# apple/ml-cvnets

Measured on NVIDIA H100. Metric: images/sec training step, MobileViTv2-1.0 bf16 256x256, higher is better.
Workload: dtype bf16

## Files before the change

### ml-cvnets_b200/csrc/gemm_tc.cu

```cuda
#include "common.cuh"
#include <cstdlib>

namespace {

constexpr int TC_BM = 128;
constexpr int TC_BN = 128;
constexpr int TC_BK = 32;
constexpr int TC_STAGE = TC_BM * TC_BK * 2;
constexpr int TC_WBLK = TC_BN * TC_BK * 2;
constexpr int TC_LDO = TC_BN + 8;
constexpr int TC_EPI_THREADS = 256;
constexpr int TC_PRODUCER_WARP = TC_EPI_THREADS / 32;
constexpr int TC_THREADS = TC_EPI_THREADS + 32;
constexpr int TC_XF_THREADS_MAX = 256;
template <int AMODE>
struct XfCfg {
  static constexpr int THREADS = (AMODE == CVB_A_RAW) ? 0 : (AMODE == CVB_A_BNB ? 128 : TC_XF_THREADS_MAX);
  static constexpr int IT = THREADS ? (TC_BM * 4) / THREADS : 1;
};
constexpr int TC_MAX_STAGES = 12;

enum { TEPI_STORE = 0, TEPI_STORE_R = 1, TEPI_SILU_BWD = 2, TEPI_GN_BWD = 3 };

__device__ __forceinline__ uint64_t desc_sw64(uint32_t saddr) { return wgmma_desc(saddr, 16, 512, WG_SW64); }
__device__ __forceinline__ void epi_bar_sync() { asm volatile("bar.sync 1, %0;" ::"n"(TC_EPI_THREADS) : "memory"); }

template <int AMODE, int EPI, bool WRES>
__global__ void __launch_bounds__(TC_THREADS + XfCfg<AMODE>::THREADS, 1)
    pw_gemm_tc_kernel(const __grid_constant__ CUtensorMap tmA, const __grid_constant__ CUtensorMap tmA2, const __grid_constant__ CUtensorMap tmW,
                      const cvb_gemm_args p, int NST) {
  constexpr bool XF = (AMODE != CVB_A_RAW);
  constexpr bool TWO_A = (AMODE == CVB_A_BNB);
  constexpr bool HAS_P = (AMODE == CVB_A_AFF || AMODE == CVB_A_AFF_SILU || AMODE == CVB_A_GN || AMODE == CVB_A_BNB);
  const int tid = threadIdx.x, lane = tid & 31, warp = tid >> 5;
  const int n0 = blockIdx.x * TC_BN;
  const int KT = (p.K + TC_BK - 1) / TC_BK;
  const int m_tiles = (p.M + TC_BM - 1) / TC_BM;
  const int my_tiles = (m_tiles - (int)blockIdx.y + (int)gridDim.y - 1) / (int)gridDim.y;
  const int total = my_tiles * KT;

  extern __shared__ __align__(1024) uint8_t smem_raw[];
  uint8_t* smem = smem_raw + ((1024u - (smem_u32(smem_raw) & 1023u)) & 1023u);
  constexpr int A_BYTES = (TWO_A ? 2 : 1) * TC_STAGE;
  constexpr int RING_STAGE = A_BYTES + (WRES ? 0 : TC_WBLK);
  uint8_t* sW = smem;
  uint8_t* sA = sW + (WRES ? KT * TC_WBLK : 0);
  uint8_t* sO = sA + NST * RING_STAGE;
  float* sP = reinterpret_cast<float*>(sO + TC_BM * TC_LDO * 2);
  __shared__ __align__(8) uint64_t full[TC_MAX_STAGES], empty[TC_MAX_STAGES], ready[TC_MAX_STAGES];
  __shared__ __align__(8) uint64_t wbar;
  __shared__ double s_samp[2][128];

  if (tid == 0) {
    for (int i = 0; i < NST; ++i) { mbar_init(&full[i], 1); mbar_init(&empty[i], 2); mbar_init(&ready[i], XfCfg<AMODE>::THREADS ? XfCfg<AMODE>::THREADS / 32 : 1); }
    mbar_init(&wbar, 1);
    fence_mbar_init();
  }
  if (tid < 128) { s_samp[0][tid] = 0.0; s_samp[1][tid] = 0.0; }
  __syncthreads();
  pdl_wait();
  pdl_trigger();

  if (warp == TC_PRODUCER_WARP) {
    if (lane == 0) {
      if (WRES) {
        mbar_expect_tx(&wbar, (uint32_t)KT * TC_WBLK);
        for (int kt = 0; kt < KT; ++kt) tma_load_2d(sW + kt * TC_WBLK, &tmW, &wbar, kt * TC_BK, n0);
      }
      for (int it = 0; it < total; ++it) {
        const int stage = it % NST;
        if (it >= NST) mbar_wait(&empty[stage], ((it / NST) - 1) & 1);
        const int j = it / KT, kt = it - j * KT;
        const int m0 = ((int)blockIdx.y + j * (int)gridDim.y) * TC_BM;
        mbar_expect_tx(&full[stage], RING_STAGE);
        tma_load_2d(sA + stage * RING_STAGE, &tmA, &full[stage], kt * TC_BK, m0);
        if (TWO_A) tma_load_2d(sA + stage * RING_STAGE + TC_STAGE, &tmA2, &full[stage], kt * TC_BK, m0);
        if (!WRES) tma_load_2d(sA + stage * RING_STAGE + A_BYTES, &tmW, &full[stage], kt * TC_BK, n0);
      }
    }
  } else if (warp > TC_PRODUCER_WARP) {
    if (XF) {
      constexpr int TC_XF_THREADS = XfCfg<AMODE>::THREADS > 0 ? XfCfg<AMODE>::THREADS : 128;
      constexpr int TC_XF_IT = XfCfg<AMODE>::IT;
      const int tt = tid - TC_THREADS;
      const int Kpad = KT * TC_BK;
      if (HAS_P) {
        for (int k = tt; k < Kpad; k += TC_XF_THREADS) {
          const bool ok = k < p.K;
          sP[k] = ok ? p.a_p0[k] : 0.f;
          sP[Kpad + k] = ok ? p.a_p1[k] : 0.f;
          if (AMODE == CVB_A_BNB) sP[2 * Kpad + k] = ok ? p.a_p2[k] : 0.f;
        }
        asm volatile("bar.sync 2, %0;" ::"n"(TC_XF_THREADS) : "memory");
      }
      float tmu[TC_XF_IT], trs[TC_XF_IT];
#pragma unroll
      for (int i = 0; i < TC_XF_IT; ++i) { tmu[i] = 0.f; trs[i] = 1.f; }
      for (int it = 0; it < total; ++it) {
        const int stage = it % NST;
        const int j = it / KT, kt = it - j * KT;
        const int m0 = ((int)blockIdx.y + j * (int)gridDim.y) * TC_BM;
        const int k0 = kt * TC_BK;
        if (AMODE == CVB_A_GN && kt == 0) {
#pragma unroll
          for (int i = 0; i < TC_XF_IT; ++i) {
            const int m = m0 + (tt >> 2) + i * (TC_XF_THREADS / 4);
            const int b = (m < p.M ? m : p.M - 1) / p.rows_per_sample;
            tmu[i] = __ldg(p.row_mean + b);
            trs[i] = __ldg(p.row_rstd + b);
          }
        }
        mbar_wait(&full[stage], (it / NST) & 1);
        uint8_t* st = sA + stage * RING_STAGE;
#pragma unroll
        for (int i = 0; i < TC_XF_IT; ++i) {
          const int c = tt + i * TC_XF_THREADS;
          const int row = c >> 2, ch = c & 3;
          const int k = k0 + ch * 8;
          const uint32_t off = (uint32_t)(row * 64 + ((ch ^ ((row >> 1) & 3)) << 4));
          uint4* pa = reinterpret_cast<uint4*>(st + off);
          float f[8], q0[8], q1[8];
          unpack8(*pa, f);
          if (HAS_P) {
            *reinterpret_cast<float4*>(q0) = *reinterpret_cast<const float4*>(sP + k);
            *reinterpret_cast<float4*>(q0 + 4) = *reinterpret_cast<const float4*>(sP + k + 4);
            *reinterpret_cast<float4*>(q1) = *reinterpret_cast<const float4*>(sP + Kpad + k);
            *reinterpret_cast<float4*>(q1 + 4) = *reinterpret_cast<const float4*>(sP + Kpad + k + 4);
          }
          if (AMODE == CVB_A_AFF) {
#pragma unroll
            for (int e = 0; e < 8; ++e) f[e] = fmaf(q0[e], f[e], q1[e]);
          } else if (AMODE == CVB_A_AFF_SILU) {
#pragma unroll
            for (int e = 0; e < 8; ++e) f[e] = silu_f(fmaf(q0[e], f[e], q1[e]));
          } else if (AMODE == CVB_A_SILU) {
#pragma unroll
            for (int e = 0; e < 8; ++e) f[e] = silu_f(f[e]);
          } else if (AMODE == CVB_A_GN) {
#pragma unroll
            for (int e = 0; e < 8; ++e) f[e] = fmaf((f[e] - tmu[i]) * trs[i], q0[e], q1[e]);
          } else if (AMODE == CVB_A_BNB) {
            float y[8], q2[8];
            unpack8(*reinterpret_cast<const uint4*>(st + TC_STAGE + off), y);
            *reinterpret_cast<float4*>(q2) = *reinterpret_cast<const float4*>(sP + 2 * Kpad + k);
            *reinterpret_cast<float4*>(q2 + 4) = *reinterpret_cast<const float4*>(sP + 2 * Kpad + k + 4);
#pragma unroll
            for (int e = 0; e < 8; ++e) f[e] = fmaf(q0[e], f[e], fmaf(q1[e], y[e], q2[e]));
          }
          *pa = (m0 + row < p.M) ? pack8(f) : make_uint4(0u, 0u, 0u, 0u);
        }
        fence_proxy_async();
        __syncwarp();
        if (lane == 0) mbar_arrive(&ready[stage]);
      }
    }
  } else {
    const int et = tid;
    const int wg = tid >> 7;
    const int r0 = wg * 64 + ((tid & 127) >> 5) * 16 + (lane >> 2);
    const int pc = 2 * (lane & 3);
    int chn[2];
    bool ch_ok[2];
    float bias[2], ep0[2], ep1[2];
#pragma unroll
    for (int h = 0; h < 2; ++h) {
      chn[h] = n0 + r0 + 8 * h;
      ch_ok[h] = chn[h] < p.N;
      bias[h] = (ch_ok[h] && p.bias) ? __ldg(p.bias + chn[h]) : 0.f;
      ep0[h] = ((EPI == TEPI_SILU_BWD || EPI == TEPI_GN_BWD) && ch_ok[h] && p.e_p0) ? __ldg(p.e_p0 + chn[h]) : 1.f;
      ep1[h] = (EPI == TEPI_SILU_BWD && ch_ok[h] && p.e_p1) ? __ldg(p.e_p1 + chn[h]) : 0.f;
    }
    constexpr bool has_aux = (EPI != TEPI_STORE);
    const bf16* __restrict__ AUX = static_cast<const bf16*>(EPI == TEPI_STORE_R ? p.R : p.Y);
    const int ldaux = EPI == TEPI_STORE_R ? p.ldr : p.ldy;
    const bool want_samp = (p.samp_sum != nullptr) && (EPI != TEPI_GN_BWD);
    const bool lin_bwd = (p.e_mode == CVB_E_LIN_BWD);
    const int rps = p.rows_per_sample > 0 ? p.rows_per_sample : 1;
    float cs[2] = {0.f, 0.f}, cq[2] = {0.f, 0.f};
    bf16* __restrict__ Cg = static_cast<bf16*>(p.C);
    constexpr int CGS = TC_BN / 8;
    const uint32_t w_off = (uint32_t)wg * 64 * 64;

    auto issue_aux = [&](int j) {
      const int m0 = ((int)blockIdx.y + j * (int)gridDim.y) * TC_BM;
      for (int c = et; c < TC_BM * CGS; c += TC_EPI_THREADS) {
        const int row = c / CGS, cgc = c % CGS;
        const int m = m0 + row, n = n0 + cgc * 8;
        const bool ok = (m < p.M) && (n < p.N);
        cp_async16(smem_u32(sO + row * (TC_LDO * 2) + cgc * 16), AUX + (ok ? (size_t)m * ldaux + n : 0), ok);
      }
      cp_async_commit();
    };
    if (has_aux && my_tiles > 0) issue_aux(0);
    if (WRES) mbar_wait(&wbar, 0);

    float acc[64];
    int it = 0;
    for (int j = 0; j < my_tiles; ++j) {
      const int m0 = ((int)blockIdx.y + j * (int)gridDim.y) * TC_BM;
      for (int kt = 0; kt < KT; ++kt, ++it) {
        const int stage = it % NST;
        mbar_wait(XF ? &ready[stage] : &full[stage], (it / NST) & 1);
        const uint32_t aa = smem_u32(sA + stage * RING_STAGE);
        const uint32_t wa = (WRES ? smem_u32(sW + kt * TC_WBLK) : aa + A_BYTES) + w_off;
        wgmma_fence();
#pragma unroll
        for (int k = 0; k < TC_BK / 16; ++k) wgmma_m64n128<0, 0>(acc, desc_sw64(wa + k * 32), desc_sw64(aa + k * 32), (kt | k) ? 1u : 0u);
        wgmma_commit();
        wgmma_wait<1>();
        if (kt > 0 && (tid & 127) == 0) mbar_arrive(&empty[(it - 1) % NST]);
      }
      wgmma_wait<0>();
      wgmma_reg_fence<64>(acc);
      if ((tid & 127) == 0) mbar_arrive(&empty[(it - 1) % NST]);

      if (has_aux) {
        cp_async_wait<0>();
        epi_bar_sync();
      }
      const bool full_tile = (m0 + TC_BM <= p.M);
      float gs[2][2] = {{0.f, 0.f}, {0.f, 0.f}}, gq[2][2] = {{0.f, 0.f}, {0.f, 0.f}};
#pragma unroll
      for (int h = 0; h < 2; ++h) {
        bf16* so = reinterpret_cast<bf16*>(sO) + r0 + 8 * h;
        if (full_tile && !has_aux) {
#pragma unroll
          for (int jb = 0; jb < 16; ++jb) {
#pragma unroll
            for (int e = 0; e < 2; ++e) {
              const float v = acc[4 * jb + 2 * h + e] + bias[h];
              so[(8 * jb + pc + e) * TC_LDO] = __float2bfloat16_rn(v);
              cs[h] += v;
              cq[h] = fmaf(v, v, cq[h]);
            }
          }
        } else {
#pragma unroll
          for (int jb = 0; jb < 16; ++jb) {
#pragma unroll
            for (int e = 0; e < 2; ++e) {
              const int i = 8 * jb + pc + e;
              float v = acc[4 * jb + 2 * h + e] + ((full_tile || m0 + i < p.M) ? bias[h] : 0.f);
              float y = 0.f;
              if (has_aux) y = __bfloat162float(so[i * TC_LDO]);
              if (EPI == TEPI_STORE_R) v += y;
              if (EPI == TEPI_SILU_BWD && !lin_bwd) v *= silu_grad_f(fmaf(ep0[h], y, ep1[h]));
              if (EPI == TEPI_GN_BWD) {
                gs[h][jb >> 3] += v;
                gq[h][jb >> 3] = fmaf(v, y, gq[h][jb >> 3]);
                so[i * TC_LDO] = __float2bfloat16_rn(v * ep0[h]);
              } else {
                const bf16 vb = __float2bfloat16_rn(v);
                so[i * TC_LDO] = vb;
                const float vr = __bfloat162float(vb);
                cs[h] += vr;
                cq[h] = fmaf(vr, EPI == TEPI_SILU_BWD ? y : vr, cq[h]);
              }
            }
          }
        }
      }
      if (EPI == TEPI_GN_BWD) {
        const int nsamples = (p.M + rps - 1) / rps;
#pragma unroll
        for (int h = 0; h < 2; ++h) {
#pragma unroll
          for (int hf = 0; hf < 2; ++hf) {
            float a = gs[h][hf], bx = gq[h][hf];
            a += __shfl_xor_sync(0xffffffffu, a, 1);
            a += __shfl_xor_sync(0xffffffffu, a, 2);
            bx += __shfl_xor_sync(0xffffffffu, bx, 1);
            bx += __shfl_xor_sync(0xffffffffu, bx, 2);
            const int mh = m0 + hf * 64;
            if ((lane & 3) == 0 && ch_ok[h] && mh < p.M) {
              double* wsA = p.gn_ws + (size_t)(mh / rps) * p.N + chn[h];
              atomicAdd(wsA, (double)a);
              atomicAdd(wsA + (size_t)nsamples * p.N, (double)bx);
            }
          }
        }
      }
      epi_bar_sync();
      const int first_sample = m0 / rps;
      for (int c = et; c < TC_BM * CGS; c += TC_EPI_THREADS) {
        const int row = c / CGS, cgc = c % CGS;
        const int m = m0 + row, n = n0 + cgc * 8;
        const uint4 u = *reinterpret_cast<const uint4*>(sO + row * (TC_LDO * 2) + cgc * 16);
        if (m < p.M && n < p.N) stg16(Cg + (size_t)m * p.ldc + n, u);
        if (want_samp) {
          float f[8];
          unpack8(u, f);
          float sv = 0.f, sq = 0.f;
#pragma unroll
          for (int e = 0; e < 8; ++e) { sv += f[e]; sq = fmaf(f[e], f[e], sq); }
#pragma unroll
          for (int o = CGS / 2; o > 0; o >>= 1) {
            sv += __shfl_xor_sync(0xffffffffu, sv, o);
            sq += __shfl_xor_sync(0xffffffffu, sq, o);
          }
          if (cgc == 0 && m < p.M) {
            atomicAdd(&s_samp[0][m / rps - first_sample], (double)sv);
            atomicAdd(&s_samp[1][m / rps - first_sample], (double)sq);
          }
        }
      }
      epi_bar_sync();
      if (want_samp) {
        const int mlast = min(m0 + TC_BM, p.M) - 1;
        const int nsamp = mlast / rps - first_sample + 1;
        if (et < nsamp) {
          atomicAdd(p.samp_sum + first_sample + et, s_samp[0][et]);
          atomicAdd(p.samp_sq + first_sample + et, s_samp[1][et]);
          s_samp[0][et] = 0.0;
          s_samp[1][et] = 0.0;
        }
      }
      if (has_aux && j + 1 < my_tiles) issue_aux(j + 1);
    }
    if (EPI != TEPI_GN_BWD) {
#pragma unroll
      for (int h = 0; h < 2; ++h) {
        float s = cs[h], q = cq[h];
        s += __shfl_xor_sync(0xffffffffu, s, 1);
        s += __shfl_xor_sync(0xffffffffu, s, 2);
        q += __shfl_xor_sync(0xffffffffu, q, 1);
        q += __shfl_xor_sync(0xffffffffu, q, 2);
        if (p.col_sum && ch_ok[h] && (lane & 3) == 0) {
          atomicAdd(p.col_sum + chn[h], (double)s);
          atomicAdd(p.col_sq + chn[h], (double)q);
        }
      }
    }
  }
}

template <int AMODE, int EPI, bool WRES>
int launch_tc_impl(const cvb_gemm_args& a, cudaStream_t st, size_t fixed, int stage_bytes) {
  const size_t budget = (size_t)216 * 1024;
  int nst = (int)((budget - fixed) / stage_bytes);
  if (nst > TC_MAX_STAGES) nst = TC_MAX_STAGES;
  const size_t smem = fixed + (size_t)nst * stage_bytes;
  static bool attr = false;
  if (!attr) {
    CVB_CUDA(cudaFuncSetAttribute(pw_gemm_tc_kernel<AMODE, EPI, WRES>, cudaFuncAttributeMaxDynamicSharedMemorySize, 216 * 1024));
    attr = true;
  }
  const int n_tiles = (a.N + TC_BN - 1) / TC_BN, m_tiles = (a.M + TC_BM - 1) / TC_BM;
  int gy = cvb_num_sms() / n_tiles;
  if (gy > m_tiles) gy = m_tiles;
  if (gy < 1) gy = 1;
  CUtensorMap tmA, tmA2, tmW;
  if (cvb_make_tmap_2d_k32(&tmA, a.A, a.M, a.K, a.lda, TC_BM)) return 1;
  if (cvb_make_tmap_2d_k32(&tmA2, AMODE == CVB_A_BNB ? a.A2 : a.A, a.M, a.K, AMODE == CVB_A_BNB ? a.lda2 : a.lda, TC_BM)) return 1;
  if (cvb_make_tmap_2d_k32(&tmW, a.W, a.N, a.K, a.ldw, TC_BN)) return 1;
  dim3 grid(n_tiles, gy);
  const int threads = TC_THREADS + XfCfg<AMODE>::THREADS;
  CVB_CUDA(cvb_launch(pw_gemm_tc_kernel<AMODE, EPI, WRES>, grid, threads, smem, st, tmA, tmA2, tmW, a, nst));
  CVB_LAUNCH_CHECK();
  return 0;
}

template <int AMODE, int EPI>
int launch_tc(const cvb_gemm_args& a, cudaStream_t st) {
  const int KT = (a.K + TC_BK - 1) / TC_BK;
  const int nvec = (AMODE == CVB_A_AFF || AMODE == CVB_A_AFF_SILU || AMODE == CVB_A_GN) ? 2 : (AMODE == CVB_A_BNB ? 3 : 0);
  const int a_bytes = (AMODE == CVB_A_BNB ? 2 : 1) * TC_STAGE;
  const size_t stagebuf = (size_t)TC_BM * TC_LDO * 2 + (size_t)nvec * KT * TC_BK * 4 + 1024;
  const size_t panel = (size_t)KT * TC_WBLK;
  if (panel + stagebuf + 6 * (size_t)a_bytes <= (size_t)216 * 1024) return launch_tc_impl<AMODE, EPI, true>(a, st, panel + stagebuf, a_bytes);
  return launch_tc_impl<AMODE, EPI, false>(a, st, stagebuf, a_bytes + TC_WBLK);
}

__global__ void __launch_bounds__(128) gn_bwd_ws_finalize_kernel(const double* __restrict__ ws, const float* __restrict__ mean,
                                                                  const float* __restrict__ rstd, const float* __restrict__ gamma, int B, int N,
                                                                  double* col_sum, double* col_sq, double* samp_sum, double* samp_sq) {
  pdl_wait();
  pdl_trigger();
  __shared__ double s_red[2][4];
  const int b = blockIdx.x, tid = threadIdx.x;
  if (b >= B) {
    __shared__ double s_col[2][8][16];
    const int cl = tid & 15, sg = tid >> 4, c = (b - B) * 16 + cl;
    double sa = 0.0, st = 0.0;
    if (c < N) {
#pragma unroll 4
      for (int s = sg; s < B; s += 8) {
        const double A = ws[(size_t)s * N + c], Bx = ws[((size_t)B + s) * N + c];
        sa += A;
        st += (double)rstd[s] * (Bx - (double)mean[s] * A);
      }
    }
    s_col[0][sg][cl] = sa;
    s_col[1][sg][cl] = st;
    __syncthreads();
    if (sg == 0 && c < N) {
      for (int g = 1; g < 8; ++g) { sa += s_col[0][g][cl]; st += s_col[1][g][cl]; }
      col_sum[c] += sa;
      col_sq[c] += st;
    }
    return;
  }
  const double mu = (double)mean[b], rs = (double)rstd[b];
  double sg = 0.0, sgx = 0.0;
  for (int c = tid; c < N; c += 128) {
    const double A = ws[(size_t)b * N + c], Bx = ws[((size_t)B + b) * N + c];
    const double t = rs * (Bx - mu * A);
    const double gm = gamma ? (double)gamma[c] : 1.0;
    sg += gm * A;
    sgx += gm * t;
  }
#pragma unroll
  for (int o = 16; o > 0; o >>= 1) {
    sg += __shfl_xor_sync(0xffffffffu, sg, o);
    sgx += __shfl_xor_sync(0xffffffffu, sgx, o);
  }
  if ((tid & 31) == 0) { s_red[0][tid >> 5] = sg; s_red[1][tid >> 5] = sgx; }
  __syncthreads();
  if (tid == 0 && samp_sum) {
    atomicAdd(samp_sum + b, s_red[0][0] + s_red[0][1] + s_red[0][2] + s_red[0][3]);
    atomicAdd(samp_sq + b, s_red[1][0] + s_red[1][1] + s_red[1][2] + s_red[1][3]);
  }
}

template <int AMODE>
int launch_tc_gn_bwd(const cvb_gemm_args& a, cudaStream_t st) {
  int rc = launch_tc<AMODE, TEPI_GN_BWD>(a, st);
  if (rc != 0) return rc;
  const int B = (a.M + a.rows_per_sample - 1) / a.rows_per_sample;
  const int col_blocks = a.col_sum ? (a.N + 15) / 16 : 0;
  CVB_CUDA(cvb_launch(gn_bwd_ws_finalize_kernel, B + col_blocks, 128, 0, st, static_cast<const double*>(a.gn_ws), a.row_mean, a.row_rstd, a.e_p0, B, a.N, a.col_sum,
                      a.col_sq, a.samp_sum, a.samp_sq));
  CVB_LAUNCH_CHECK();
  return 0;
}

template <int AMODE>
int dispatch_tc_epi(const cvb_gemm_args& a, cudaStream_t st) {
  if (a.e_mode == CVB_E_GN_BWD && a.gn_ws && a.rows_per_sample % (TC_BM / 2) == 0 && !a.bias && (AMODE == CVB_A_RAW || AMODE == CVB_A_BNB))
    return launch_tc_gn_bwd<AMODE == CVB_A_BNB ? CVB_A_BNB : CVB_A_RAW>(a, st);
  if (a.e_mode == CVB_E_STORE) return a.R ? launch_tc<AMODE, TEPI_STORE_R>(a, st) : launch_tc<AMODE, TEPI_STORE>(a, st);
  if ((a.e_mode == CVB_E_SILU_BWD || a.e_mode == CVB_E_LIN_BWD) && (AMODE == CVB_A_RAW || AMODE == CVB_A_BNB)) return launch_tc<AMODE == CVB_A_BNB ? CVB_A_BNB : CVB_A_RAW, TEPI_SILU_BWD>(a, st);
  return -1;
}

}

int cvb_pw_gemm_tc(const cvb_gemm_args& a, cudaStream_t st) {
  static const int min_n = [] { const char* e = getenv("CVB_TC_MIN_N"); return e ? atoi(e) : 96; }();
  if (a.N < min_n || (a.N >= 96 && a.N % 128 != 0 && a.N % 128 < 64 && a.N < 256)) return -1;
  switch (a.a_mode) {
    case CVB_A_RAW: return dispatch_tc_epi<CVB_A_RAW>(a, st);
    case CVB_A_AFF: return dispatch_tc_epi<CVB_A_AFF>(a, st);
    case CVB_A_AFF_SILU: return dispatch_tc_epi<CVB_A_AFF_SILU>(a, st);
    case CVB_A_SILU: return dispatch_tc_epi<CVB_A_SILU>(a, st);
    case CVB_A_GN: return dispatch_tc_epi<CVB_A_GN>(a, st);
    case CVB_A_BNB: return dispatch_tc_epi<CVB_A_BNB>(a, st);
    default: return -1;
  }
}
```

### ml-cvnets_b200/csrc/norm.cu

```cuda
#include <stdarg.h>

#include "common.cuh"

static thread_local char g_err[512] = "";
void cvb_set_error(const char* fmt, ...) {
  va_list ap;
  va_start(ap, fmt);
  vsnprintf(g_err, sizeof(g_err), fmt, ap);
  va_end(ap);
}
extern "C" const char* cvb_last_error(void) { return g_err; }
extern "C" int cvb_abi_version(void) { return CVB_ABI_VERSION; }
static int g_pdl_enabled = 1;
int cvb_pdl_enabled() { return g_pdl_enabled; }
extern "C" int cvb_set_pdl_enabled(int on) {
  int old = g_pdl_enabled;
  g_pdl_enabled = on ? 1 : 0;
  return old;
}

int cvb_num_sms() {
  static int sms = 0;
  if (sms == 0) {
    int dev = 0;
// ... 435 lines not shown
    const float mu = mean[row], rs = rstd[row];
    float v[LNB_MAXCH][8], xh[LNB_MAXCH][8];
    uint4 dres[LNB_MAXCH];
    float s1 = 0.f, s2 = 0.f;
#pragma unroll
    for (int q = 0; q < LNB_MAXCH; ++q) {
      const int ch = lane + 32 * q;
      if (ch < nch) {
        unpack8(ldg16_stream(V + row * C + ch * 8), v[q]);
        unpack8(ldg16_stream(X + row * C + ch * 8), xh[q]);
        if (DRES) dres[q] = ldg16_stream(DRES + row * C + ch * 8);
      }
    }
#pragma unroll
    for (int q = 0; q < LNB_MAXCH; ++q) {
      const int ch = lane + 32 * q;
      if (ch < nch) {
        float gq[8];
        *reinterpret_cast<float4*>(gq) = *reinterpret_cast<const float4*>(sgam + ch * 8);
        *reinterpret_cast<float4*>(gq + 4) = *reinterpret_cast<const float4*>(sgam + ch * 8 + 4);
#pragma unroll
        for (int e = 0; e < 8; ++e) {
          xh[q][e] = (xh[q][e] - mu) * rs;
          atomicAdd(&sred[e * nch + ch], v[q][e]);
          atomicAdd(&sred[C + e * nch + ch], v[q][e] * xh[q][e]);
          v[q][e] *= gq[e];
          s1 += v[q][e];
          s2 = fmaf(v[q][e], xh[q][e], s2);
        }
      }
    }
    s1 = warp_sum(s1) * invC;
    s2 = warp_sum(s2) * invC;
#pragma unroll
    for (int q = 0; q < LNB_MAXCH; ++q) {
      const int ch = lane + 32 * q;
      if (ch < nch) {
        float d[8];
        if (DRES) unpack8(dres[q], d);
#pragma unroll
        for (int e = 0; e < 8; ++e) {
          float o = rs * (v[q][e] - s1 - xh[q][e] * s2);
          if (DRES) o += d[e];
          d[e] = o;
          if (col_sum) atomicAdd(&sred[2 * C + e * nch + ch], o);
        }
        stg16(DX + row * C + ch * 8, pack8(d));
      }
    }
  }
  __syncthreads();
  for (int i = tid; i < C; i += NT) {
    const int t = (i & 7) * (C / 8) + (i >> 3);
    atomicAdd(dbeta + i, (double)sred[t]);
    atomicAdd(dgamma + i, (double)sred[C + t]);
    if (col_sum) atomicAdd(col_sum + i, (double)sred[2 * C + t]);
  }
}

__device__ __forceinline__ float act_fwd_f(float x, int kind) {
  switch (kind) {
    case 0: return silu_f(x);
    case 1: return 0.5f * x * (1.0f + erff(x * 0.70710678118654752f));
    case 2: return fmaxf(x, 0.f);
    case 3: return x * fminf(fmaxf(x + 3.0f, 0.f), 6.0f) * (1.0f / 6.0f);
    case 4: return fminf(fmaxf(x + 3.0f, 0.f), 6.0f) * (1.0f / 6.0f);
    default: return 1.0f / (1.0f + __expf(-x));
  }
}
__device__ __forceinline__ float act_grad_f(float x, int kind) {
  switch (kind) {
    case 0: return silu_grad_f(x);
    case 1: {
      const float cdf = 0.5f * (1.0f + erff(x * 0.70710678118654752f));
      return cdf + x * 0.3989422804014327f * __expf(-0.5f * x * x);
    }
    case 2: return x > 0.f ? 1.f : 0.f;
    case 3: return x <= -3.0f ? 0.f : (x < 3.0f ? fmaf(x, 1.0f / 3.0f, 0.5f) : 1.0f);
    case 4: return (x > -3.0f && x < 3.0f) ? (1.0f / 6.0f) : 0.f;
    default: {
      const float s = 1.0f / (1.0f + __expf(-x));
      return s * (1.0f - s);
    }
  }
}
__global__ void __launch_bounds__(NT) act_fwd_kernel(const bf16* __restrict__ X, bf16* __restrict__ Y, int64_t nvec, int kind) {
  pdl_wait();
  pdl_trigger();
  for (int64_t v = (int64_t)blockIdx.x * NT + threadIdx.x; v < nvec; v += (int64_t)gridDim.x * NT) {
    float f[8];
    unpack8(ldg16_stream(X + v * 8), f);
#pragma unroll
    for (int j = 0; j < 8; ++j) f[j] = act_fwd_f(f[j], kind);
    stg16(Y + v * 8, pack8(f));
  }
}
__global__ void __launch_bounds__(NT) act_bwd_kernel(const bf16* __restrict__ DY, const bf16* __restrict__ X, bf16* __restrict__ DX, int64_t nvec,
                                                     int kind) {
  pdl_wait();
  pdl_trigger();
  for (int64_t v = (int64_t)blockIdx.x * NT + threadIdx.x; v < nvec; v += (int64_t)gridDim.x * NT) {
    float g[8], x[8];
    unpack8(ldg16_stream(DY + v * 8), g);
    unpack8(ldg16_stream(X + v * 8), x);
#pragma unroll
    for (int j = 0; j < 8; ++j) g[j] *= act_grad_f(x[j], kind);
    stg16(DX + v * 8, pack8(g));
  }
}

__global__ void __launch_bounds__(NT) ln_stats_kernel(const bf16* __restrict__ X, int ldx, int64_t M, int C, float eps, float* __restrict__ mean,
                                                      float* __restrict__ rstd) {
  pdl_wait();
  pdl_trigger();
  const int lane = threadIdx.x & 31;
  const int64_t row = (int64_t)blockIdx.x * (NT / 32) + (threadIdx.x >> 5);
  if (row >= M) return;
  const bf16* x = X + row * ldx;
  float s = 0.f, q = 0.f;
  for (int c = lane * 8; c < C; c += 256) {
    float f[8];
    unpack8(ldg16(x + c), f);
#pragma unroll
    for (int e = 0; e < 8; ++e) { s += f[e]; q = fmaf(f[e], f[e], q); }
  }
  s = warp_sum(s);
  q = warp_sum(q);
  if (lane == 0) {
    const float mu = s / (float)C;
    float var = q / (float)C - mu * mu;
    if (var < 0.f) var = 0.f;
    mean[row] = mu;
    rstd[row] = rsqrtf(var + eps);
  }
}

__global__ void __launch_bounds__(NT) gn_bwd_apply_kernel(const bf16* __restrict__ G, const bf16* __restrict__ X, const float* __restrict__ mean,
                                                          const float* __restrict__ rstd, const double* __restrict__ sg, const double* __restrict__ sgx,
                                                          double count, const bf16* __restrict__ DRES, bf16* __restrict__ DX, int64_t M,
                                                          int rows_per_sample, int C, double* col_sum, int cgs, int rpp, int rows_per_cta,
                                                          const float* __restrict__ gamma) {
  pdl_wait();
  pdl_trigger();
  extern __shared__ double sdred[];
  const int tid = threadIdx.x;
  if (col_sum) { for (int i = tid; i < C; i += blockDim.x) sdred[i] = 0.0; __syncthreads(); }
  const int cg = tid % cgs, rr = tid / cgs;
  const int c = cg * 8;
  float a0[8], gm[8];
#pragma unroll
  for (int j = 0; j < 8; ++j) { a0[j] = 0.f; gm[j] = gamma ? gamma[c + j] : 1.0f; }
  int64_t r_begin = (int64_t)blockIdx.x * rows_per_cta, r_end = r_begin + rows_per_cta;
  if (r_end > M) r_end = M;
  for (int64_t r = r_begin + rr; r < r_end; r += rpp) {
    const int b = (int)(r / rows_per_sample);
    const float mu = mean[b], rs = rstd[b];
    const float m1 = (float)(sg[b] / count), m2 = (float)(sgx[b] / count);
    float g[8], x[8];
    unpack8(ldg16_stream(G + r * C + c), g);
    unpack8(ldg16_stream(X + r * C + c), x);
#pragma unroll
    for (int j = 0; j < 8; ++j) {
      float xh = (x[j] - mu) * rs;
      g[j] = rs * (g[j] * gm[j] - m1 - xh * m2);
    }
    if (DRES) {
      float d[8];
      unpack8(ldg16_stream(DRES + r * C + c), d);
#pragma unroll
      for (int j = 0; j < 8; ++j) g[j] += d[j];
    }
#pragma unroll
    for (int j = 0; j < 8; ++j) a0[j] += g[j];
    stg16(DX + r * C + c, pack8(g));
  }
  if (col_sum) {
#pragma unroll
    for (int j = 0; j < 8; ++j) atomicAdd(&sdred[c + j], (double)a0[j]);
    __syncthreads();
    for (int i = tid; i < C; i += blockDim.x) atomicAdd(col_sum + i, sdred[i]);
  }
}

__global__ void __launch_bounds__(NT) pool_fwd_kernel(const bf16* __restrict__ X, int HW, int C, bf16* __restrict__ OUT) {
  pdl_wait();
  pdl_trigger();
  extern __shared__ double sdred[];
  const int b = blockIdx.x;
  const int cgs = C / 8;
  const int tid = threadIdx.x;
  for (int i = tid; i < C; i += blockDim.x) sdred[i] = 0.0;
  __syncthreads();
  const int cg = tid % cgs, rr = tid / cgs, rpp = blockDim.x / cgs;
  float a[8];
#pragma unroll
  for (int j = 0; j < 8; ++j) a[j] = 0.f;
  for (int r = rr; r < HW; r += rpp) {
    float f[8];
    unpack8(ldg16(X + ((int64_t)b * HW + r) * C + cg * 8), f);
#pragma unroll
    for (int j = 0; j < 8; ++j) a[j] += f[j];
  }
#pragma unroll
  for (int j = 0; j < 8; ++j) atomicAdd(&sdred[cg * 8 + j], (double)a[j]);
  __syncthreads();
  for (int i = tid; i < C; i += blockDim.x) OUT[(int64_t)b * C + i] = __float2bfloat16_rn((float)sdred[i] / (float)HW);
}

__global__ void __launch_bounds__(NT) pool_bwd_kernel(const bf16* __restrict__ DOUT, int HW, int C, bf16* __restrict__ DX, int64_t nvec) {
  pdl_wait();
  pdl_trigger();
  const int cgs = C / 8;
  const float inv = 1.f / (float)HW;
  for (int64_t v = (int64_t)blockIdx.x * NT + threadIdx.x; v < nvec; v += (int64_t)gridDim.x * NT) {
    int64_t row = v / cgs;
    int c = (int)(v % cgs) * 8;
    int64_t b = row / HW;
    float f[8];
    unpack8(ldg16(DOUT + b * C + c), f);
#pragma unroll
    for (int j = 0; j < 8; ++j) f[j] *= inv;
    stg16(DX + v * 8, pack8(f));
  }
}

__global__ void __launch_bounds__(NT) stem_im2col_kernel(const float* __restrict__ X, int64_t sxn, int64_t sxc, int64_t sxh, int64_t sxw, int B, int H,
                                                         int W, bf16* __restrict__ A, const float* __restrict__ mix) {
  pdl_wait();
  pdl_trigger();
  const int Ho = H / 2, Wo = W / 2;
  const int mode = mix ? (int)mix[0] : 0;
  const float lam = mix ? mix[1] : 1.f;
  const int bx1 = mix ? (int)mix[2] : 0, by1 = mix ? (int)mix[3] : 0, bx2 = mix ? (int)mix[4] : 0, by2 = mix ? (int)mix[5] : 0;
  const int64_t total = (int64_t)B * Ho * Wo * 4;
  for (int64_t i = (int64_t)blockIdx.x * NT + threadIdx.x; i < total; i += (int64_t)gridDim.x * NT) {
    const int ch = (int)(i & 3);
    const int64_t pix = i >> 2;
    const int ow = (int)(pix % Wo);
    const int oh = (int)((pix / Wo) % Ho);
    const int b = (int)(pix / ((int64_t)Wo * Ho));
    float f[8];
#pragma unroll
    for (int j = 0; j < 8; ++j) {
      const int col = ch * 8 + j;
      float v = 0.f;
      if (col < 27) {
        const int ci = col / 9, u = (col % 9) / 3, vv = col % 3;
        const int h = 2 * oh + u - 1, w = 2 * ow + vv - 1;
        if (h >= 0 && h < H && w >= 0 && w < W) {
          const int64_t off = ci * sxc + h * sxh + w * sxw;
          v = __ldg(X + b * sxn + off);
          if (mode != 0) {
            const int bp = b == 0 ? B - 1 : b - 1;
            if (mode == 1) v = fmaf(lam, v, (1.0f - lam) * __ldg(X + bp * sxn + off));
            else if (h >= by1 && h < by2 && w >= bx1 && w < bx2) v = __ldg(X + bp * sxn + off);
          }
        }
      }
      f[j] = v;
    }
    stg16(A + i * 8, pack8(f));
  }
}

__device__ __forceinline__ int perm_row(int r, int rows, int rot) { return rot ? (r + rot) % rows : r; }

__global__ void __launch_bounds__(NT) prep_weights_kernel(const cvb_prep_desc* __restrict__ descs) {
  pdl_wait();
  pdl_trigger();
  const cvb_prep_desc d = descs[blockIdx.y];
  const int64_t total = (d.kind == 2) ? (int64_t)d.rows * d.cols : (d.kind == 3 ? (int64_t)d.dst_rows : (int64_t)d.dst_rows * d.ldd);
  for (int64_t i = (int64_t)blockIdx.x * NT + threadIdx.x; i < total; i += (int64_t)gridDim.x * NT) {
    if (d.kind == 0) {
      int r = (int)(i / d.ldd), c = (int)(i % d.ldd);
      float v = (r < d.rows && c < d.cols) ? d.src[(int64_t)perm_row(r, d.rows, d.rot) * d.cols + c] : 0.f;
      static_cast<bf16*>(d.dst)[i] = __float2bfloat16_rn(v);
    } else if (d.kind == 1) {
      int c = (int)(i / d.ldd), r = (int)(i % d.ldd);
      float v = (r < d.rows && c < d.cols) ? d.src[(int64_t)perm_row(r, d.rows, d.rot) * d.cols + c] : 0.f;
      static_cast<bf16*>(d.dst)[i] = __float2bfloat16_rn(v);
    } else if (d.kind == 2) {
      int tap = (int)(i / d.rows), ch = (int)(i % d.rows);
      static_cast<float*>(d.dst)[i] = bf16_round(d.src[(int64_t)ch * d.cols + tap]);
    } else if (d.kind == 4 || d.kind == 5) {
      const int r = (d.kind == 4) ? (int)(i / d.ldd) : (int)(i % d.ldd), c = (d.kind == 4) ? (int)(i % d.ldd) : (int)(i / d.ldd);
      const int cin = d.cols / d.rot;
      float v = 0.f;
      if (r < d.rows && c < d.cols) v = d.src[(int64_t)r * d.cols + (c % cin) * d.rot + c / cin];
      static_cast<bf16*>(d.dst)[i] = __float2bfloat16_rn(v);
    } else {
      int r = (int)i;
      static_cast<float*>(d.dst)[i] = (r < d.rows) ? d.src[perm_row(r, d.rows, d.rot)] : 0.f;
    }
  }
}

__global__ void __launch_bounds__(NT) unprep_grad_kernel(const float* __restrict__ src, float* __restrict__ dst, int rows, int cols, int lds, int kind,
                                                         int rot) {
  pdl_wait();
  pdl_trigger();
  const int64_t total = (int64_t)rows * cols;
  for (int64_t i = (int64_t)blockIdx.x * NT + threadIdx.x; i < total; i += (int64_t)gridDim.x * NT) {
    if (kind == 0) {
      int r = (int)(i / cols), c = (int)(i % cols);
      dst[(int64_t)perm_row(r, rows, rot) * cols + c] = src[(int64_t)r * lds + c];
    } else if (kind == 2) {
      int ch = (int)(i / cols), tap = (int)(i % cols);
      dst[i] = src[(int64_t)tap * rows + ch];
    } else if (kind == 4) {
      int r = (int)(i / cols), c = (int)(i % cols);
      const int cin = cols / rot;
      dst[(int64_t)r * cols + (c % cin) * rot + c / cin] = src[(int64_t)r * lds + c];
    } else {
      dst[perm_row((int)i, rows, rot)] = src[i];
    }
  }
}

int grid_for(int64_t n_items) {
  int64_t g = (n_items + NT - 1) / NT;
  int64_t cap = 16 * (int64_t)cvb_num_sms();
  if (g > cap) g = cap;
  if (g < 1) g = 1;
  return (int)g;
}

}

// ... 226 lines not shown
```

Measured before the change: 6882.

## Add 64-row tile variant of pointwise GEMM with two CTAs per SM

Templates the tensor-core pointwise GEMM on the pixel tile height, adding a 64-row variant that uses m64n64 wgmma, half the accumulators, a halved shared-memory budget and two CTAs per SM. Light epilogue GEMMs whose weight panel fits resident now take this path, aiming to improve SM fill and latency hiding on small or skinny problems. Separately, the GroupNorm backward apply kernel is unrolled four rows deep so loads are batched ahead of the math, increasing memory-level parallelism. The smaller tile gives each CTA fewer pipeline stages and less weight reuse per CTA.

```diff
diff --git a/ml-cvnets_b200/csrc/gemm_tc.cu b/ml-cvnets_b200/csrc/gemm_tc.cu
--- a/ml-cvnets_b200/csrc/gemm_tc.cu
+++ b/ml-cvnets_b200/csrc/gemm_tc.cu
@@ -3,32 +3,35 @@
 
 namespace {
 
-constexpr int TC_BM = 128;
 constexpr int TC_BN = 128;
 constexpr int TC_BK = 32;
-constexpr int TC_STAGE = TC_BM * TC_BK * 2;
 constexpr int TC_WBLK = TC_BN * TC_BK * 2;
 constexpr int TC_LDO = TC_BN + 8;
 constexpr int TC_EPI_THREADS = 256;
 constexpr int TC_PRODUCER_WARP = TC_EPI_THREADS / 32;
 constexpr int TC_THREADS = TC_EPI_THREADS + 32;
-constexpr int TC_XF_THREADS_MAX = 256;
-template <int AMODE>
+template <int AMODE, int BM>
 struct XfCfg {
-  static constexpr int THREADS = (AMODE == CVB_A_RAW) ? 0 : (AMODE == CVB_A_BNB ? 128 : TC_XF_THREADS_MAX);
-  static constexpr int IT = THREADS ? (TC_BM * 4) / THREADS : 1;
+  static constexpr int THREADS = (AMODE == CVB_A_RAW) ? 0 : (BM == 64 ? 32 : (AMODE == CVB_A_BNB ? 128 : 256));
+  static constexpr int IT = THREADS ? (BM * 4) / THREADS : 1;
 };
 constexpr int TC_MAX_STAGES = 12;
+constexpr size_t TC_SMEM_1CTA = (size_t)216 * 1024;
+constexpr size_t TC_SMEM_2CTA = (size_t)108 * 1024;
 
 enum { TEPI_STORE = 0, TEPI_STORE_R = 1, TEPI_SILU_BWD = 2, TEPI_GN_BWD = 3 };
 
 __device__ __forceinline__ uint64_t desc_sw64(uint32_t saddr) { return wgmma_desc(saddr, 16, 512, WG_SW64); }
 __device__ __forceinline__ void epi_bar_sync() { asm volatile("bar.sync 1, %0;" ::"n"(TC_EPI_THREADS) : "memory"); }
 
-template <int AMODE, int EPI, bool WRES>
-__global__ void __launch_bounds__(TC_THREADS + XfCfg<AMODE>::THREADS, 1)
+template <int AMODE, int EPI, bool WRES, int BM>
+__global__ void __launch_bounds__(TC_THREADS + XfCfg<AMODE, BM>::THREADS, BM == 64 ? 2 : 1)
     pw_gemm_tc_kernel(const __grid_constant__ CUtensorMap tmA, const __grid_constant__ CUtensorMap tmA2, const __grid_constant__ CUtensorMap tmW,
                       const cvb_gemm_args p, int NST) {
+  static_assert(BM == 128 || BM == 64, "pixel tile is 128 or 64");
+  constexpr int TC_BM = BM;
+  constexpr int TC_STAGE = TC_BM * TC_BK * 2;
+  constexpr int NACC = TC_BM / 2;
   constexpr bool XF = (AMODE != CVB_A_RAW);
   constexpr bool TWO_A = (AMODE == CVB_A_BNB);
   constexpr bool HAS_P = (AMODE == CVB_A_AFF || AMODE == CVB_A_AFF_SILU || AMODE == CVB_A_GN || AMODE == CVB_A_BNB);
@@ -49,14 +52,14 @@
   float* sP = reinterpret_cast<float*>(sO + TC_BM * TC_LDO * 2);
   __shared__ __align__(8) uint64_t full[TC_MAX_STAGES], empty[TC_MAX_STAGES], ready[TC_MAX_STAGES];
   __shared__ __align__(8) uint64_t wbar;
-  __shared__ double s_samp[2][128];
+  __shared__ double s_samp[2][TC_BM];
 
   if (tid == 0) {
-    for (int i = 0; i < NST; ++i) { mbar_init(&full[i], 1); mbar_init(&empty[i], 2); mbar_init(&ready[i], XfCfg<AMODE>::THREADS ? XfCfg<AMODE>::THREADS / 32 : 1); }
+    for (int i = 0; i < NST; ++i) { mbar_init(&full[i], 1); mbar_init(&empty[i], 2); mbar_init(&ready[i], XfCfg<AMODE, BM>::THREADS ? XfCfg<AMODE, BM>::THREADS / 32 : 1); }
     mbar_init(&wbar, 1);
     fence_mbar_init();
   }
-  if (tid < 128) { s_samp[0][tid] = 0.0; s_samp[1][tid] = 0.0; }
+  if (tid < TC_BM) { s_samp[0][tid] = 0.0; s_samp[1][tid] = 0.0; }
   __syncthreads();
   pdl_wait();
   pdl_trigger();
@@ -80,8 +83,8 @@
     }
   } else if (warp > TC_PRODUCER_WARP) {
     if (XF) {
-      constexpr int TC_XF_THREADS = XfCfg<AMODE>::THREADS > 0 ? XfCfg<AMODE>::THREADS : 128;
-      constexpr int TC_XF_IT = XfCfg<AMODE>::IT;
+      constexpr int TC_XF_THREADS = XfCfg<AMODE, BM>::THREADS > 0 ? XfCfg<AMODE, BM>::THREADS : 128;
+      constexpr int TC_XF_IT = XfCfg<AMODE, BM>::IT;
       const int tt = tid - TC_THREADS;
       const int Kpad = KT * TC_BK;
       if (HAS_P) {
@@ -194,7 +197,7 @@
     if (has_aux && my_tiles > 0) issue_aux(0);
     if (WRES) mbar_wait(&wbar, 0);
 
-    float acc[64];
+    float acc[NACC];
     int it = 0;
     for (int j = 0; j < my_tiles; ++j) {
       const int m0 = ((int)blockIdx.y + j * (int)gridDim.y) * TC_BM;
@@ -205,13 +208,16 @@
         const uint32_t wa = (WRES ? smem_u32(sW + kt * TC_WBLK) : aa + A_BYTES) + w_off;
         wgmma_fence();
 #pragma unroll
-        for (int k = 0; k < TC_BK / 16; ++k) wgmma_m64n128<0, 0>(acc, desc_sw64(wa + k * 32), desc_sw64(aa + k * 32), (kt | k) ? 1u : 0u);
+        for (int k = 0; k < TC_BK / 16; ++k) {
+          if constexpr (TC_BM == 128) wgmma_m64n128<0, 0>(acc, desc_sw64(wa + k * 32), desc_sw64(aa + k * 32), (kt | k) ? 1u : 0u);
+          else wgmma_m64n64<0, 0>(acc, desc_sw64(wa + k * 32), desc_sw64(aa + k * 32), (kt | k) ? 1u : 0u);
+        }
         wgmma_commit();
         wgmma_wait<1>();
         if (kt > 0 && (tid & 127) == 0) mbar_arrive(&empty[(it - 1) % NST]);
       }
       wgmma_wait<0>();
-      wgmma_reg_fence<64>(acc);
+      wgmma_reg_fence<NACC>(acc);
       if ((tid & 127) == 0) mbar_arrive(&empty[(it - 1) % NST]);
 
       if (has_aux) {
@@ -225,7 +231,7 @@
         bf16* so = reinterpret_cast<bf16*>(sO) + r0 + 8 * h;
         if (full_tile && !has_aux) {
 #pragma unroll
-          for (int jb = 0; jb < 16; ++jb) {
+          for (int jb = 0; jb < TC_BM / 8; ++jb) {
 #pragma unroll
             for (int e = 0; e < 2; ++e) {
               const float v = acc[4 * jb + 2 * h + e] + bias[h];
@@ -236,7 +242,7 @@
           }
         } else {
 #pragma unroll
-          for (int jb = 0; jb < 16; ++jb) {
+          for (int jb = 0; jb < TC_BM / 8; ++jb) {
 #pragma unroll
             for (int e = 0; e < 2; ++e) {
               const int i = 8 * jb + pc + e;
@@ -265,7 +271,7 @@
 #pragma unroll
         for (int h = 0; h < 2; ++h) {
 #pragma unroll
-          for (int hf = 0; hf < 2; ++hf) {
+          for (int hf = 0; hf < TC_BM / 64; ++hf) {
             float a = gs[h][hf], bx = gq[h][hf];
             a += __shfl_xor_sync(0xffffffffu, a, 1);
             a += __shfl_xor_sync(0xffffffffu, a, 2);
@@ -334,41 +340,61 @@
   }
 }
 
-template <int AMODE, int EPI, bool WRES>
+template <int AMODE, int EPI, bool WRES, int BM>
 int launch_tc_impl(const cvb_gemm_args& a, cudaStream_t st, size_t fixed, int stage_bytes) {
-  const size_t budget = (size_t)216 * 1024;
+  constexpr int CTAS_PER_SM = BM == 64 ? 2 : 1;
+  constexpr size_t budget = BM == 64 ? TC_SMEM_2CTA : TC_SMEM_1CTA;
   int nst = (int)((budget - fixed) / stage_bytes);
   if (nst > TC_MAX_STAGES) nst = TC_MAX_STAGES;
   const size_t smem = fixed + (size_t)nst * stage_bytes;
   static bool attr = false;
   if (!attr) {
-    CVB_CUDA(cudaFuncSetAttribute(pw_gemm_tc_kernel<AMODE, EPI, WRES>, cudaFuncAttributeMaxDynamicSharedMemorySize, 216 * 1024));
+    CVB_CUDA(cudaFuncSetAttribute(pw_gemm_tc_kernel<AMODE, EPI, WRES, BM>, cudaFuncAttributeMaxDynamicSharedMemorySize, (int)budget));
+    CVB_CUDA(cudaFuncSetAttribute(pw_gemm_tc_kernel<AMODE, EPI, WRES, BM>, cudaFuncAttributePreferredSharedMemoryCarveout, cudaSharedmemCarveoutMaxShared));
     attr = true;
   }
-  const int n_tiles = (a.N + TC_BN - 1) / TC_BN, m_tiles = (a.M + TC_BM - 1) / TC_BM;
-  int gy = cvb_num_sms() / n_tiles;
+  const int n_tiles = (a.N + TC_BN - 1) / TC_BN, m_tiles = (a.M + BM - 1) / BM;
+  int gy = CTAS_PER_SM * cvb_num_sms() / n_tiles;
   if (gy > m_tiles) gy = m_tiles;
   if (gy < 1) gy = 1;
   CUtensorMap tmA, tmA2, tmW;
-  if (cvb_make_tmap_2d_k32(&tmA, a.A, a.M, a.K, a.lda, TC_BM)) return 1;
-  if (cvb_make_tmap_2d_k32(&tmA2, AMODE == CVB_A_BNB ? a.A2 : a.A, a.M, a.K, AMODE == CVB_A_BNB ? a.lda2 : a.lda, TC_BM)) return 1;
+  if (cvb_make_tmap_2d_k32(&tmA, a.A, a.M, a.K, a.lda, BM)) return 1;
+  if (cvb_make_tmap_2d_k32(&tmA2, AMODE == CVB_A_BNB ? a.A2 : a.A, a.M, a.K, AMODE == CVB_A_BNB ? a.lda2 : a.lda, BM)) return 1;
   if (cvb_make_tmap_2d_k32(&tmW, a.W, a.N, a.K, a.ldw, TC_BN)) return 1;
   dim3 grid(n_tiles, gy);
-  const int threads = TC_THREADS + XfCfg<AMODE>::THREADS;
-  CVB_CUDA(cvb_launch(pw_gemm_tc_kernel<AMODE, EPI, WRES>, grid, threads, smem, st, tmA, tmA2, tmW, a, nst));
+  const int threads = TC_THREADS + XfCfg<AMODE, BM>::THREADS;
+  CVB_CUDA(cvb_launch(pw_gemm_tc_kernel<AMODE, EPI, WRES, BM>, grid, threads, smem, st, tmA, tmA2, tmW, a, nst));
   CVB_LAUNCH_CHECK();
   return 0;
 }
 
+struct TcSmem {
+  size_t stagebuf, panel, budget;
+  int a_bytes;
+  bool wres() const { return panel + stagebuf + 6 * (size_t)a_bytes <= budget; }
+};
+template <int AMODE, int BM>
+TcSmem tc_smem(int K) {
+  const int KT = (K + TC_BK - 1) / TC_BK;
+  const int nvec = (AMODE == CVB_A_AFF || AMODE == CVB_A_AFF_SILU || AMODE == CVB_A_GN) ? 2 : (AMODE == CVB_A_BNB ? 3 : 0);
+  return {(size_t)BM * TC_LDO * 2 + (size_t)nvec * KT * TC_BK * 4 + 1024, (size_t)KT * TC_WBLK, BM == 64 ? TC_SMEM_2CTA : TC_SMEM_1CTA,
+          (AMODE == CVB_A_BNB ? 2 : 1) * BM * TC_BK * 2};
+}
+
+template <int AMODE, int EPI, int BM>
+int launch_tc_bm(const cvb_gemm_args& a, cudaStream_t st) {
+  const TcSmem s = tc_smem<AMODE, BM>(a.K);
+  if (s.wres()) return launch_tc_impl<AMODE, EPI, true, BM>(a, st, s.panel + s.stagebuf, s.a_bytes);
+  return launch_tc_impl<AMODE, EPI, false, BM>(a, st, s.stagebuf, s.a_bytes + TC_WBLK);
+}
+
 template <int AMODE, int EPI>
 int launch_tc(const cvb_gemm_args& a, cudaStream_t st) {
-  const int KT = (a.K + TC_BK - 1) / TC_BK;
-  const int nvec = (AMODE == CVB_A_AFF || AMODE == CVB_A_AFF_SILU || AMODE == CVB_A_GN) ? 2 : (AMODE == CVB_A_BNB ? 3 : 0);
-  const int a_bytes = (AMODE == CVB_A_BNB ? 2 : 1) * TC_STAGE;
-  const size_t stagebuf = (size_t)TC_BM * TC_LDO * 2 + (size_t)nvec * KT * TC_BK * 4 + 1024;
-  const size_t panel = (size_t)KT * TC_WBLK;
-  if (panel + stagebuf + 6 * (size_t)a_bytes <= (size_t)216 * 1024) return launch_tc_impl<AMODE, EPI, true>(a, st, panel + stagebuf, a_bytes);
-  return launch_tc_impl<AMODE, EPI, false>(a, st, stagebuf, a_bytes + TC_WBLK);
+  constexpr bool light = (AMODE == CVB_A_RAW || AMODE == CVB_A_SILU) && (EPI == TEPI_STORE || EPI == TEPI_STORE_R);
+  if constexpr (light) {
+    if (a.col_sum == nullptr && tc_smem<AMODE, 128>(a.K).wres()) return launch_tc_bm<AMODE, EPI, 64>(a, st);
+  }
+  return launch_tc_bm<AMODE, EPI, 128>(a, st);
 }
 
 __global__ void __launch_bounds__(128) gn_bwd_ws_finalize_kernel(const double* __restrict__ ws, const float* __restrict__ mean,
@@ -436,7 +462,7 @@
 
 template <int AMODE>
 int dispatch_tc_epi(const cvb_gemm_args& a, cudaStream_t st) {
-  if (a.e_mode == CVB_E_GN_BWD && a.gn_ws && a.rows_per_sample % (TC_BM / 2) == 0 && !a.bias && (AMODE == CVB_A_RAW || AMODE == CVB_A_BNB))
+  if (a.e_mode == CVB_E_GN_BWD && a.gn_ws && a.rows_per_sample % 64 == 0 && !a.bias && (AMODE == CVB_A_RAW || AMODE == CVB_A_BNB))
     return launch_tc_gn_bwd<AMODE == CVB_A_BNB ? CVB_A_BNB : CVB_A_RAW>(a, st);
   if (a.e_mode == CVB_E_STORE) return a.R ? launch_tc<AMODE, TEPI_STORE_R>(a, st) : launch_tc<AMODE, TEPI_STORE>(a, st);
   if ((a.e_mode == CVB_E_SILU_BWD || a.e_mode == CVB_E_LIN_BWD) && (AMODE == CVB_A_RAW || AMODE == CVB_A_BNB)) return launch_tc<AMODE == CVB_A_BNB ? CVB_A_BNB : CVB_A_RAW, TEPI_SILU_BWD>(a, st);
diff --git a/ml-cvnets_b200/csrc/norm.cu b/ml-cvnets_b200/csrc/norm.cu
--- a/ml-cvnets_b200/csrc/norm.cu
+++ b/ml-cvnets_b200/csrc/norm.cu
@@ -611,28 +611,48 @@
   for (int j = 0; j < 8; ++j) { a0[j] = 0.f; gm[j] = gamma ? gamma[c + j] : 1.0f; }
   int64_t r_begin = (int64_t)blockIdx.x * rows_per_cta, r_end = r_begin + rows_per_cta;
   if (r_end > M) r_end = M;
-  for (int64_t r = r_begin + rr; r < r_end; r += rpp) {
-    const int b = (int)(r / rows_per_sample);
-    const float mu = mean[b], rs = rstd[b];
-    const float m1 = (float)(sg[b] / count), m2 = (float)(sgx[b] / count);
-    float g[8], x[8];
-    unpack8(ldg16_stream(G + r * C + c), g);
-    unpack8(ldg16_stream(X + r * C + c), x);
-#pragma unroll
-    for (int j = 0; j < 8; ++j) {
-      float xh = (x[j] - mu) * rs;
-      g[j] = rs * (g[j] * gm[j] - m1 - xh * m2);
-    }
-    if (DRES) {
-      float d[8];
-      unpack8(ldg16_stream(DRES + r * C + c), d);
-#pragma unroll
-      for (int j = 0; j < 8; ++j) g[j] += d[j];
-    }
-#pragma unroll
-    for (int j = 0; j < 8; ++j) a0[j] += g[j];
-    stg16(DX + r * C + c, pack8(g));
-  }
+  constexpr int U = 4;
+  auto rows = [&](int64_t r, int n) {
+    uint4 ug[U], ux[U], ud[U];
+#pragma unroll
+    for (int u = 0; u < U; ++u) {
+      if (u < n) {
+        const int64_t o = (r + (int64_t)u * rpp) * C + c;
+        ug[u] = ldg16_stream(G + o);
+        ux[u] = ldg16_stream(X + o);
+        if (DRES) ud[u] = ldg16_stream(DRES + o);
+      }
+    }
+#pragma unroll
+    for (int u = 0; u < U; ++u) {
+      if (u < n) {
+        const int64_t ru = r + (int64_t)u * rpp;
+        const int b = (int)(ru / rows_per_sample);
+        const float mu = mean[b], rs = rstd[b];
+        const float m1 = (float)(sg[b] / count), m2 = (float)(sgx[b] / count);
+        float g[8], x[8];
+        unpack8(ug[u], g);
+        unpack8(ux[u], x);
+#pragma unroll
+        for (int j = 0; j < 8; ++j) {
+          float xh = (x[j] - mu) * rs;
+          g[j] = rs * (g[j] * gm[j] - m1 - xh * m2);
+        }
+        if (DRES) {
+          float d[8];
+          unpack8(ud[u], d);
+#pragma unroll
+          for (int j = 0; j < 8; ++j) g[j] += d[j];
+        }
+#pragma unroll
+        for (int j = 0; j < 8; ++j) a0[j] += g[j];
+        stg16(DX + ru * C + c, pack8(g));
+      }
+    }
+  };
+  int64_t r = r_begin + rr;
+  for (; r + (int64_t)(U - 1) * rpp < r_end; r += (int64_t)U * rpp) rows(r, U);
+  if (r < r_end) rows(r, (int)((r_end - r + rpp - 1) / rpp));
   if (col_sum) {
 #pragma unroll
     for (int j = 0; j < 8; ++j) atomicAdd(&sdred[c + j], (double)a0[j]);
```

New measurement: 6948 (median of 6 runs). No clear change (+1.0%).
